# katehai/m-cedm

Hardware: AMD Instinct MI355X
Metric: denoised_states_per_sec_18step_edm_heun (higher is better)
Workload: dtype f32; 1 GPU; SWE-periodic 128x128, EDM U-Net ch=128 ch_mult=[1,1,1,1] attn@16^2 (BASELINE config 3); states_per_gpu=32, global_batch=32, H=128, W=128, sampler=EDM Heun, 18 steps, 35 NFE/state, S_churn=0, w=0, fp64 state / fp32 net, parallelism=batch-sharded x1, no data-path collective, launch=one HIP graph per sampler call

## Files before the change

### include/mcedm_hip.h

```cpp
#ifndef MCEDM_HIP_H_
#define MCEDM_HIP_H_

#include <stddef.h>
#include <stdint.h>

#ifdef __cplusplus
extern "C" {
#endif

#define MCEDM_ABI_VERSION 4
#define MCEDM_REDUCE_SCRATCH_BYTES (4096 * 8 + 64)
#define MCEDM_MAX_LEVELS 8

typedef enum {
  MCEDM_OK = 0,
  MCEDM_ERR_INVALID = -1,
  MCEDM_ERR_UNSUPPORTED = -2,
  MCEDM_ERR_WORKSPACE = -3,
  MCEDM_ERR_HIP = -4
} mcedm_status;

#define MCEDM_DX_NONE 0
#define MCEDM_DX_CAT 1
#define MCEDM_DX_ENC 2
// ... 155 lines not shown
                         const float* init_noise, const double* step_noise, double* out, int return_last, void* workspace,
                         size_t workspace_bytes, int B, int H, int W, void* stream);
int mcedm_vp_heun_sample_rng(const mcedm_plan* plan, const void* packed, const mcedm_vp_sampler_desc* sp, const float* cond,
                             const float* init_noise, const uint64_t* rng_seed, double* out, int return_last, void* workspace,
                             size_t workspace_bytes, int B, int H, int W, void* stream);


typedef struct { float mean, scale, offset, pad; } mcedm_coef;

size_t mcedm_op_conv_packed_floats(int Cout, int Cin, int k);
int mcedm_op_pack_conv(const float* w, const float* b, int Cout, int Cin, int k, int qkv_heads, int dgrad,
                       float* wpk, float* bias_pk, void* stream);
int mcedm_op_gn_coef(const float* xa, const float* xb, int Ca, int Cb, int B, int HW, const float* gamma,
                     const float* beta, const float* film, int film_batch, int film_stride, float eps,
                     mcedm_coef* coef_out, float* stats_out, void* stream);
int mcedm_op_conv(const float* xa, const float* xb, int Ca, int Cb, const mcedm_coef* coef, int coef_batch, int act,
                  int resample, int Hs, int Ws, int H, int W, const float* wpk, const float* bias_pk,
                  const float* res, int res_mode, float* out, int Cout, int B, int k, void* stream);
size_t mcedm_op_conv_wino_packed_floats(int Cout, int Cin);
int mcedm_op_pack_conv_wino(const float* w, int Cout, int Cin, float* wino, void* stream);
int mcedm_op_conv_wino(const float* xa, const float* xb, int Ca, int Cb, const mcedm_coef* coef, int coef_batch, int act,
                       int resample, int H, int W, const float* wino, const float* bias, const float* res, int res_mode,
                       float* out, int Cout, int B, void* stream);
int mcedm_op_embedding(const float* labels, int n, int ch, const float* w0, const float* b0, const float* w1,
                       const float* b1, const float* waff, const float* baff, int rows, float* freqs_scratch,
                       float* emb_out, float* film_out, void* stream);
int mcedm_op_attention(const float* qkv, float* out, int B, int heads, int T, void* stream);
size_t mcedm_op_wgrad_scratch_floats(int Cout, int Cin, int k, int B, int H, int W);
int mcedm_op_conv_wgrad(const float* dy, const float* xa, const float* xb, int Ca, int Cb, const mcedm_coef* coef,
                        int coef_batch, int act, int resample, int Hs, int Ws, int H, int W, int Cout, int B, int k,
                        int qkv_heads, float* scratch, float* dw, float* db, void* stream);
int mcedm_op_gn_bwd(const float* dact, int resample, const float* xa, const float* xb, int Ca, int Cb, int Hs, int Ws,
                    int B, const mcedm_coef* coef, const float* stats, const float* gamma, const float* beta,
                    const float* film, int film_batch, int film_stride, int act, float* dxa, float* dxb, int accumulate,
                    const float* add, int add_mode, float* ab, float* dgamma, float* dbeta, float* dfilm,
                    int dfilm_stride, void* stream);
#define MCEDM_GN_SYNC_WORDS 130
int mcedm_op_gn_bwd_sync(const float* dact, int resample, const float* xa, const float* xb, int Ca, int Cb, int Hs, int Ws,
                         int B, const mcedm_coef* coef, const float* stats, const float* gamma, const float* beta,
                         const float* film, int film_batch, int film_stride, int act, float* dxa, float* dxb, int accumulate,
                         const float* add, int add_mode, float* ab, float* dgamma, float* dbeta, float* dfilm,
                         int dfilm_stride, unsigned int* sync, void* stream);
int mcedm_op_attention_bwd(const float* qkv, const float* a, const float* da, float* dqkv, float* lse_scratch, int B,
                           int heads, int T, void* stream);
int mcedm_op_set_conv_tile(int mt, int ph, int pw);
int mcedm_op_set_conv8(int enable);
int mcedm_op_set_conv_resident(int enable);
int mcedm_op_set_conv_wino(int enable);
int mcedm_op_set_conv_wino1(int enable);
int mcedm_op_set_wgrad_wino(int enable);
int mcedm_op_set_conv1x1_reg(int enable);
int mcedm_op_set_attn_fused(int enable);
int mcedm_op_set_conv_debug(unsigned long long* buf);

typedef struct {
  int32_t in_channels;
  int32_t out_channels;
  int32_t ch;
  int32_t n_levels;
  int32_t ch_mult[MCEDM_MAX_LEVELS];
  int32_t num_res_blocks;
  int32_t resolution;
  int32_t n_attn_resolutions;
  int32_t attn_resolutions[MCEDM_MAX_LEVELS];
  int32_t self_cond;
  float eps;
} mcedm_ddpm_desc;

typedef struct {
  int32_t timesteps;
  double sigma_min, sigma_max, rho;
  double S_churn, S_min, S_max, S_noise;
// ... 65 lines not shown
```

### m-cedm_amd/csrc/conv_wino.hip

```cpp
#include <atomic>
#include <cstdlib>

#include "conv_wino.hpp"
#include "pack.hpp"
#include "prof.hpp"

namespace mcedm {

__global__ void wino_pack_kernel(const float* __restrict__ w, float* __restrict__ dst, int Cout, int Cin, int coutp, int nch,
                                 int tflip) {
  const int idx = blockIdx.x * blockDim.x + threadIdx.x;
  if (idx >= coutp * nch * WKC) return;
  wino_pack_elem(w, dst, idx, Cout, Cin, coutp, tflip);
}

template <class C, bool UP, bool ACT = true>
__global__ __launch_bounds__(C::NT, C::MB == 4 ? 1 : 2) void conv_wino_kernel(const ConvArgs p, int tiles_x, int tiles_img, int nch, int mblocks,
                                                                          int per, int mode) {
  constexpr int WSC = C::SC, VBUF = C::VBUF, RBUF = C::RBUF, MB = C::MB;
  extern __shared__ float lds[];
  const int Cin = p.Ca + p.Cb;
  float* const vbuf = lds;
  float* const rbuf = lds + 2 * VBUF;
  Coef* const cfl = reinterpret_cast<Coef*>(lds + C::LDS_ROWS_OFF);
  float* const xch = lds + C::LDS_ROWS_OFF + 4 * Cin;
  float* const red = xch + C::XCH_FLOATS;
  float* const bias_l = red + 2 * (C::MT / 2) * 3;
  const int tid = threadIdx.x, lane = tid & 63;
  const int wave = __builtin_amdgcn_readfirstlane(tid >> 6);
  const int mb = wave % MB, hf = wave / MB;
  if (p.dbg && tid == 0) { p.dbg[blockIdx.x * 16 + 0] = __builtin_amdgcn_s_memrealtime(); p.dbg[blockIdx.x * 16 + 4] = per; }
  int gt0 = blockIdx.x * per, tstep = 1;
  int n = gt0 / tiles_img, tile0 = gt0 % tiles_img;
  if (mode & 256) {
    const int nwg = gridDim.x, wps = tiles_img / per;
    const int lid = (nwg % 8 == 0) ? (int)(blockIdx.x % 8) * (nwg / 8) + (int)(blockIdx.x / 8) : (int)blockIdx.x;
    n = lid / wps; tile0 = lid % wps; tstep = wps;
  }
  const int m0 = blockIdx.y * C::MT;
  const size_t HW = (size_t)p.H * p.W, HWs = (size_t)p.Hs * p.Ws;
  const int nst = (nch + WSC - 1) / WSC;
// ... 109 lines not shown
        const float* b = rb + sc * WKC * RPLANE + 2 * MB * ti * RPITCH + 2 * j;
        td[sc][ti][0][j] = *reinterpret_cast<const f32x2*>(b + tr_yz);
        td[sc][ti][1][j] = *reinterpret_cast<const f32x2*>(b + tr_yz + RPITCH);
        td[sc][ti][2][j] = *reinterpret_cast<const f32x2*>(b + tr_x);
      }
  };
  auto transform_finish1 = [&](int sc, float* vb) {
#pragma unroll
    for (int ti = 0; ti < C::TI; ++ti) {
      f32x2 t[2][2];
#pragma unroll
      for (int j = 0; j < 2; ++j) {
        t[0][j] = td[sc][ti][0][j] - td[sc][ti][2][j];
        t[1][j] = td[sc][ti][2][j] + tsgn * td[sc][ti][1][j];
      }
#pragma unroll
      for (int x = 0; x < 2; ++x) {
        const f32x2 o03 = t[x][0] - t[x][1];
        const f32x2 c11 = {t[x][0].y, t[x][0].y}, c22 = {t[x][1].x, t[x][1].x};
        const f32x2 o12 = c11 + tpm * c22;
        float* o = vb + sc * 16 * VPOS + tr_dst + MB * ti * WTX * 4 + 4 * x * VPOS;
        o[0 * VPOS] = o03.x;
        o[1 * VPOS] = o12.x;
        o[2 * VPOS] = o12.y;
        o[3 * VPOS] = o03.y;
      }
    }
  };
  auto transform_read = [&](const float* rb) { for (int sc = 0; sc < WSC; ++sc) transform_read1(sc, rb); };
  auto transform_finish = [&](float* vb) { for (int sc = 0; sc < WSC; ++sc) transform_finish1(sc, vb); };

  stage_coef_rows<C::NT>(p, n, cfl, tid);
  if (tid < C::MT) bias_l[tid] = p.bias ? p.bias[m0 + tid] : 0.f;
  raw_load();
  __syncthreads();
  for (int sc = 0; sc < WSC; ++sc) raw_commit1(sc, rbuf);
  commit_done();
  if (G > 1) { raw_load(); for (int sc = 0; sc < WSC; ++sc) raw_commit1(sc, rbuf + RBUF); commit_done(); }
  if (G > 2) raw_load();
  const size_t ustride = (size_t)mblocks * 16 * 64;
  const f32x4* up = reinterpret_cast<const f32x4*>(p.wino) + ((size_t)(m0 / 32 + mb) * 16 + 8 * hf) * 64 + lane;
  f32x4 ua[8];
#pragma unroll
  for (int q = 0; q < 8; ++q) ua[q] = up[q * 64];
  __syncthreads();
  transform_read(rbuf);
  transform_finish(vbuf);
  f32x16 acc[8];
  auto init_acc = [&]() {
    const f32x16 zero16 = {0.f, 0.f, 0.f, 0.f, 0.f, 0.f, 0.f, 0.f, 0.f, 0.f, 0.f, 0.f, 0.f, 0.f, 0.f, 0.f};
    float z = 0.f;
#pragma unroll
    for (int q = 0; q < 8; ++q) {
      asm volatile("" : "+v"(z));
      acc[q] = __builtin_amdgcn_mfma_f32_32x32x2f32(z, z, zero16, 0, 0, 0);
    }
    if (hf == 0) {
#pragma unroll
      for (int r = 0; r < 16; ++r) acc[5][r] = bias_l[32 * mb + 4 * (lane >> 5) + (r & 3) + 8 * (r >> 2)];
    }
  };
  __syncthreads();
  init_acc();

  const int vrd = (8 * hf) * VPOS + (lane >> 5) * VH1 + (lane & 31) * 4;
  if (p.dbg && tid == 0) { p.dbg[blockIdx.x * 16 + 1] = __builtin_amdgcn_s_memrealtime(); p.dbg[blockIdx.x * 16 + 5] = __builtin_amdgcn_s_memtime(); }
#ifdef MCEDM_WINO_TIMELINE
  unsigned long long ph[5] = {0, 0, 0, 0, 0}, tlast = __builtin_amdgcn_s_memtime();
#define WINO_STAMP(i) { const unsigned long long t_ = __builtin_amdgcn_s_memtime(); ph[i] += t_ - tlast; tlast = t_; }
  unsigned long long sl[8] = {0, 0, 0, 0, 0, 0, 0, 0}, slast = 0;
#define WINO_SLOT(i) { const unsigned long long t_ = __builtin_amdgcn_s_memtime(); sl[(i) & 7] += t_ - slast; slast = t_; }
#define WINO_SLOT0 { slast = __builtin_amdgcn_s_memtime(); }
  unsigned long long ep[6] = {0, 0, 0, 0, 0, 0}, elast = 0;
#define WINO_EP(i) { __builtin_amdgcn_sched_barrier(0); const unsigned long long t_ = __builtin_amdgcn_s_memtime(); if (i) ep[(i) - 1] += t_ - elast; elast = t_; __builtin_amdgcn_sched_barrier(0); }
  const bool no_u = mode & 2;
#else
#define WINO_STAMP(i)
#define WINO_SLOT(i)
#define WINO_SLOT0
#define WINO_EP(i)
  constexpr bool no_u = false;
#endif
  auto side_slice = [&](int slot, int g, int cur) {
    if (WSC == 2) {
      if (slot == 0) transform_read1(0, rbuf + (cur ^ 1) * RBUF);
      if (slot == 1) raw_commit1(0, rbuf + cur * RBUF);
      if (slot == 2) { transform_finish1(0, vbuf + (cur ^ 1) * VBUF); raw_load1(0); }
      if (slot == 3) transform_read1(WSC - 1, rbuf + (cur ^ 1) * RBUF);
      if (slot == 4) { raw_commit1(WSC - 1, rbuf + cur * RBUF); commit_done(); }
      if (slot == 5) { transform_finish1(WSC - 1, vbuf + (cur ^ 1) * VBUF); raw_load1(WSC - 1); raw_load_done(); }
    } else {
      if (slot == 0) transform_read(rbuf + (cur ^ 1) * RBUF);
      if (slot == 1) { raw_commit1(0, rbuf + cur * RBUF); commit_done(); }
      if (slot == 2) { raw_load1(0); raw_load_done(); }
      if (slot == 3) transform_finish1(0, vbuf + (cur ^ 1) * VBUF);
    }
  };
  (void)mode;
  int st = 0, tile = tile0;
  for (int g = 0; g < G; ++g) {
    const int cur = g & 1;
    WINO_STAMP(0)
    WINO_SLOT0
#pragma unroll
    for (int sc = 0; sc < WSC; ++sc) {
      const int c = st * WSC + sc;
      const f32x4* un = up + (size_t)(c + 1 < nch ? c + 1 : 0) * ustride;
      const float* vb = vbuf + cur * VBUF + sc * 16 * VPOS + vrd;
      f32x4 b4[2][2];
      b4[0][0] = *reinterpret_cast<const f32x4*>(vb);
      b4[0][1] = *reinterpret_cast<const f32x4*>(vb + VPOS);
      __builtin_amdgcn_sched_group_barrier(0x100, 2, 0);
#pragma unroll
      for (int qp = 0; qp < 4; ++qp) {
        const int cb = qp & 1;
        if (qp < 3) {
          b4[cb ^ 1][0] = *reinterpret_cast<const f32x4*>(vb + (2 * qp + 2) * VPOS);
          b4[cb ^ 1][1] = *reinterpret_cast<const f32x4*>(vb + (2 * qp + 3) * VPOS);
        }
#pragma unroll
        for (int s = 0; s < 4; ++s) {
          acc[2 * qp] = __builtin_amdgcn_mfma_f32_32x32x2f32(ua[2 * qp][s], b4[cb][0][s], acc[2 * qp], 0, 0, 0);
          acc[2 * qp + 1] = __builtin_amdgcn_mfma_f32_32x32x2f32(ua[2 * qp + 1][s], b4[cb][1][s], acc[2 * qp + 1], 0, 0, 0);
        }
        if (!no_u) {
          ua[2 * qp] = un[(2 * qp) * 64];
          ua[2 * qp + 1] = un[(2 * qp + 1) * 64];
        }
        side_slice(sc * 4 + qp, g, cur);
        if (qp < 3) __builtin_amdgcn_sched_group_barrier(0x100, 2, 0);
#pragma unroll
        for (int i = 0; i < 8; ++i) {
          __builtin_amdgcn_sched_group_barrier(0x008, 1, 0);
          __builtin_amdgcn_sched_group_barrier(0x486, WINO_IL_K, 0);
        }
        __builtin_amdgcn_sched_group_barrier(0x020, 4, 0);
        __builtin_amdgcn_sched_barrier(0);
        if (sc * 4 + qp == (WSC == 2 ? 5 : 2)) raw_load_next();
        __builtin_amdgcn_sched_barrier(0);
        WINO_SLOT(sc * 4 + qp + (WSC == 1 ? 0 : 0))
      }
    }
    WINO_STAMP(1)
    __syncthreads();
    WINO_STAMP(2)
    if (++st < nst) continue;
    st = 0;

    WINO_EP(0)
    const int y0 = (tile / tiles_x) * WPH, x0 = (tile % tiles_x) * WPW;
    const int pt = lane & 31;
    const int oy = y0 + 2 * (pt >> 3) + hf, ox = x0 + 2 * (pt & 7);
    const int cbase = m0 + 32 * mb + 4 * (lane >> 5);
    const size_t splane = (size_t)p.Cout * HW;
    const __amdgpu_buffer_rsrc_t rs_out = make_rsrc(p.out + (size_t)n * splane, 4u * (unsigned)splane);
    const size_t rplane = p.res_mode == RS_UP ? splane >> 2 : p.res_mode == RS_DOWN ? splane << 2 : splane;
    const __amdgpu_buffer_rsrc_t rs_res = make_rsrc(p.res ? p.res + (size_t)n * rplane : nullptr, p.res ? 4u * (unsigned)rplane : 0u);
    const unsigned HWu = (unsigned)HW;
    const unsigned voff = 4u * ((unsigned)cbase * HWu + (unsigned)oy * p.W + ox);
    const unsigned rvoff = 4u * ((unsigned)cbase * (HWu >> 2) + (unsigned)(oy >> 1) * (p.W >> 1) + (ox >> 1));
    float2 rv[16];
    f32x16 keep[2], send[2];
#pragma unroll
    for (int j = 0; j < 2; ++j) {
      const f32x16 t0 = j == 0 ? acc[0] + acc[1] + acc[2] : acc[1] - acc[2] - acc[3];
      const f32x16 t1 = j == 0 ? acc[4] + acc[5] + acc[6] : acc[5] - acc[6] - acc[7];
      if (hf == 0) { keep[j] = t0 + t1; send[j] = t1; }
      else         { keep[j] = -t0 - t1; send[j] = t0; }
      __builtin_amdgcn_sched_barrier(0);
    }
    __builtin_amdgcn_sched_barrier(0);
    if (p.res && p.res_mode == RS_DOWN) {
      const unsigned dvoff = 4u * ((unsigned)cbase * (HWu << 2) + (unsigned)(2 * oy) * (unsigned)(2 * p.W) + (unsigned)(2 * ox));
#pragma unroll
      for (int r0 = 0; r0 < 16; r0 += 4) {
        f32x4 ta[4], tb[4];
#pragma unroll
        for (int k = 0; k < 4; ++k) {
          const unsigned so = 4u * (unsigned)(((r0 + k) & 3) + 8 * ((r0 + k) >> 2)) * (HWu << 2);
          ta[k] = __builtin_bit_cast(f32x4, __builtin_amdgcn_raw_buffer_load_b128(rs_res, dvoff, so, 0));
          tb[k] = __builtin_bit_cast(f32x4, __builtin_amdgcn_raw_buffer_load_b128(rs_res, dvoff + 8u * (unsigned)p.W, so, 0));
        }
#pragma unroll
        for (int k = 0; k < 4; ++k)
          rv[r0 + k] = make_float2(0.25f * ((ta[k][0] + ta[k][1]) + (tb[k][0] + tb[k][1])), 0.25f * ((ta[k][2] + ta[k][3]) + (tb[k][2] + tb[k][3])));
      }
    } else {
#pragma unroll
      for (int r = 0; r < 16; ++r) {
// ... 63 lines not shown
        }
      }
      __syncthreads();
      conv_stats_store<C, 2>(p, red, n, m0, tile, tiles_img, tid);
    }
    WINO_EP(4)
    __builtin_amdgcn_sched_barrier(0);
    init_acc();
    tile += tstep;
    WINO_EP(5)
    WINO_STAMP(3)
  }
  if (p.dbg && tid == 0) {
    asm volatile("s_waitcnt vmcnt(0)" ::: "memory");
    p.dbg[blockIdx.x * 16 + 2] = __builtin_amdgcn_s_memrealtime(); p.dbg[blockIdx.x * 16 + 6] = __builtin_amdgcn_s_memtime();
    p.dbg[blockIdx.x * 16 + 3] = __builtin_amdgcn_s_memrealtime();
  }
#ifdef MCEDM_WINO_TIMELINE
  if (p.dbg && tid == 0) for (int i = 0; i < 5; ++i) p.dbg[blockIdx.x * 16 + 8 + i] = ph[i];
  if (p.dbg && tid == 0 && (mode & 16)) for (int i = 0; i < 8; ++i) p.dbg[blockIdx.x * 16 + 8 + i] = sl[i];
  if (p.dbg && tid == 0 && (mode & 32)) for (int i = 0; i < 6; ++i) p.dbg[blockIdx.x * 16 + 8 + i] = ep[i];
  if (p.dbg && tid == 64 * MB && !(mode & 48)) { p.dbg[blockIdx.x * 16 + 13] = ph[1]; p.dbg[blockIdx.x * 16 + 14] = ph[2]; p.dbg[blockIdx.x * 16 + 15] = ph[3]; p.dbg[blockIdx.x * 16 + 7] = ph[0]; }
#endif
}

static int g_wino = -1;
void set_conv_wino(int enable) { g_wino = enable; }
static int wino_env() {
  static int env = -1;
  if (env < 0) { const char* e = getenv("MCEDM_WINOGRAD"); env = e ? atoi(e) : 1; }
  return variant_choice(KV_CONV_WINO, g_wino, env);
}
static int wino_mode_env() {
  static int env = -1;
  if (env < 0) {
    const char* e = getenv("MCEDM_WINO_MODE");
    const char* m = getenv("MCEDM_WINO_MAP");
    env = ((e ? atoi(e) : 0) & ~256) | ((m ? atoi(m) : 1) ? 256 : 0);
  }
  return env;
}

static int wino_min_hw_env() {
  static int env = -1;
  if (env < 0) { const char* e = getenv("MCEDM_WINO_MIN_HW"); env = e ? atoi(e) : 1024; }
  return env;
// ... 29 lines not shown
  return best;
}

template <class C>
static int launch_wino_cfg(const ConvArgs& a, hipStream_t stream) {
  const int tiles_x = a.W / WPW, tiles_img = tiles_x * (a.H / WPH);
  const long long total = (long long)a.B * tiles_img;
  MCEDM_REQUIRE(total > 0 && total <= 0x7fffffffLL, "conv_wino: grid out of range");
  const int Cin = a.Ca + a.Cb, nch = Cin / WKC;
  const int lds_bytes = (C::LDS_ROWS_OFF + 4 * Cin + C::XCH_FLOATS + C::RED_FLOATS) * 4;
  MCEDM_REQUIRE(lds_bytes <= 160 * 1024 / (C::MB == 4 ? 1 : 2), "conv_wino: %d input channels exceed the LDS row table", Cin);
  static std::atomic<bool> attr_set[64];
  static std::atomic<int> ncu[64];
  int dev = 0;
  MCEDM_HIP_TRY(hipGetDevice(&dev));
  MCEDM_REQUIRE(dev >= 0 && dev < 64, "device index %d out of range", dev);
  if (!attr_set[dev].load(std::memory_order_acquire)) {
    int n_cu = 0;
    MCEDM_HIP_TRY(hipDeviceGetAttribute(&n_cu, hipDeviceAttributeMultiprocessorCount, dev));
    ncu[dev].store(n_cu > 0 ? n_cu : 256, std::memory_order_release);
    MCEDM_HIP_TRY(hipFuncSetAttribute((const void*)conv_wino_kernel<C, false>, hipFuncAttributeMaxDynamicSharedMemorySize, 160 * 1024));
    MCEDM_HIP_TRY(hipFuncSetAttribute((const void*)conv_wino_kernel<C, true>, hipFuncAttributeMaxDynamicSharedMemorySize, 160 * 1024));
    MCEDM_HIP_TRY(hipFuncSetAttribute((const void*)conv_wino_kernel<C, false, false>, hipFuncAttributeMaxDynamicSharedMemorySize, 160 * 1024));
    attr_set[dev].store(true, std::memory_order_release);
  }
  static int per_env = -1;
  if (per_env < 0) { const char* e = getenv("MCEDM_WINO_PER"); per_env = e ? atoi(e) : 0; }
  int per = wino_tiles_per_wg(total, tiles_img, ncu[dev].load(std::memory_order_acquire) * (C::MB == 4 ? 1 : 2));
  if (per_env > 0 && tiles_img % per_env == 0) per = per_env;
  char name[64] = "";
  const bool noact = a.resample != RS_UP && !a.act;
  if (prof_enabled()) snprintf(name, sizeof(name), "conv_wino_kernel<WinoCfg<%d>, %s, %s>", C::MB, a.resample == RS_UP ? "true" : "false",
                               noact ? "false" : "true");
  const double px = (double)a.B * a.H * a.W;
  ProfScope ps(name, 2.0 * px * a.Cout * (double)Cin * 9,
               4.0 * ((double)a.B * Cin * a.Hs * a.Ws + px * a.Cout * (a.res ? 2 : 1) + (double)a.Cout * Cin * 9), stream);
  if (a.resample == RS_UP)
    hipLaunchKernelGGL((conv_wino_kernel<C, true>), dim3((unsigned)(total / per), a.Cout / C::MT), dim3(C::NT), lds_bytes, stream, a, tiles_x,
                       tiles_img, nch, cout_padded(a.Cout) / 32, per, wino_mode_env());
  else if (noact)
    hipLaunchKernelGGL((conv_wino_kernel<C, false, false>), dim3((unsigned)(total / per), a.Cout / C::MT), dim3(C::NT), lds_bytes, stream, a, tiles_x,
                       tiles_img, nch, cout_padded(a.Cout) / 32, per, wino_mode_env());
  else
    hipLaunchKernelGGL((conv_wino_kernel<C, false>), dim3((unsigned)(total / per), a.Cout / C::MT), dim3(C::NT), lds_bytes, stream, a, tiles_x,
                       tiles_img, nch, cout_padded(a.Cout) / 32, per, wino_mode_env());
  MCEDM_LAUNCH_CHECK("conv_wino_kernel");
  if (a.gsum_tiles) *a.gsum_tiles = SumTiles{tiles_img, tiles_x, WPH, WPW, a.gsum_rc == 2 ? 2 : 4};
  return MCEDM_OK;
}

int launch_conv_wino(const ConvArgs& a_in, hipStream_t stream) {
  ConvArgs a = a_in;
  a.dbg = conv_debug_buffer();
  MCEDM_REQUIRE(conv_wino_applicable(a, 9), "conv_wino: shape not served by the Winograd kernel");
  MCEDM_REQUIRE(a.out && a.B > 0 && (a.resample == RS_UP ? (a.Hs * 2 == a.H && a.Ws * 2 == a.W) : (a.Hs == a.H && a.Ws == a.W)),
                "conv_wino: bad arguments");
  MCEDM_REQUIRE((unsigned long long)a.H * a.W * 4ull * a.Cout * (a.res && a.res_mode == RS_DOWN ? 4 : 1) < (1ull << 32),
                "conv_wino: one sample of the output / residual exceeds the 4 GiB buffer range");
  { const int rc = conv_resolve_identity(a); if (rc != MCEDM_OK) return rc; }
  if (a.Cout % 128 == 0) {
// ... 13 lines not shown
```

### m-cedm_amd/csrc/conv_wino.hpp

```cpp
#pragma once
#include "conv_tile.hpp"

namespace mcedm {

constexpr int WPH = 8, WPW = 16;
constexpr int WTX = WPW / 2, WTY = WPH / 2;
constexpr int WKC = 8;
static_assert(WTX * WTY == 32, "one MFMA N block of patches per workgroup");
template <int MB_>
struct WinoCfg {
  static constexpr int MB = MB_, NT = 128 * MB_, NW = 2 * MB_, MT = 32 * MB_;
  static constexpr int SC = MB_ == 4 ? 2 : 1;
  static constexpr int CPW = WKC / NW;
  static constexpr int TI = 4 / MB_;
  static constexpr int VBUF = SC * 16 * 288, RBUF = SC * WKC * 196;
  static constexpr int LDS_ROWS_OFF = 2 * VBUF + 2 * RBUF;
  static constexpr int XCH_FLOATS = NW * 16 * 64;
  static constexpr int RED_FLOATS = 2 * (MT / 2) * 3 + MT;
  static_assert(MB_ == 4 || MB_ == 2, "128 or 64 output channels per workgroup");
  static_assert(LDS_ROWS_OFF % 4 == 0, "LDS layout");
};
constexpr int RROWS = WPH + 2, RPITCH = WPW + 2;
constexpr int RPLANE = 196;
constexpr int RSUB = (RROWS * RPITCH + 63) / 64;
constexpr int WINO_IL_K = 5;
constexpr int VH1 = 144, VPOS = 288;
static_assert(RPLANE % 32 == 4 && VH1 % 32 == 16 && VH1 >= 128 && VPOS >= VH1 + 128 && RPLANE >= RROWS * RPITCH && RPLANE % 2 == 0 && VPOS % 4 == 0 && VH1 % 4 == 0, "LDS layout");



int try_launch_conv_wino1(const ConvArgs& a, hipStream_t stream);
void set_conv_wino1(int enable);
int wino_tiles_per_wg(long long total, int tiles_img, int slots);

}
```

### m-cedm_amd/csrc/ops_api.hip

```cpp
#include "common.hpp"
#include "conv_wino.hpp"
#include "bwd.hpp"

using namespace mcedm;

static_assert(sizeof(mcedm_coef) == sizeof(Coef), "mcedm_coef must mirror Coef");

extern "C" size_t mcedm_op_conv_packed_floats(int Cout, int Cin, int k) {
  if (Cout <= 0 || Cin <= 0 || (k != 1 && k != 3)) return 0;
  return conv_packed_floats(Cout, Cin, k * k);
}

extern "C" int mcedm_op_pack_conv(const float* w, const float* b, int Cout, int Cin, int k, int qkv_heads, int dgrad,
                                  float* wpk, float* bias_pk, void* stream) {
  MCEDM_REQUIRE(w && wpk, "op_pack_conv: null pointer");
  MCEDM_REQUIRE(Cout > 0 && Cin > 0 && (k == 1 || k == 3), "op_pack_conv: bad shape");
  MCEDM_REQUIRE(qkv_heads == 0 || (Cout % (3 * qkv_heads) == 0 && !dgrad), "op_pack_conv: bad qkv_heads");
  int rc = dgrad ? launch_pack_conv(w, wpk, Cin, Cout, k * k, 0, 1, (hipStream_t)stream)
                 : launch_pack_conv(w, wpk, Cout, Cin, k * k, qkv_heads, 0, (hipStream_t)stream);
  if (rc) return rc;
  if (b && bias_pk) rc = launch_pack_bias(b, bias_pk, Cout, qkv_heads, (hipStream_t)stream);
  return rc;
}

// ... 10 lines not shown
}

extern "C" int mcedm_op_conv(const float* xa, const float* xb, int Ca, int Cb, const mcedm_coef* coef, int coef_batch,
                             int act, int resample, int Hs, int Ws, int H, int W, const float* wpk,
                             const float* bias_pk, const float* res, int res_mode, float* out, int Cout, int B, int k,
                             void* stream) {
  MCEDM_REQUIRE(k == 1 || k == 3, "op_conv: k must be 1 or 3");
  MCEDM_REQUIRE(resample >= 0 && resample <= 3 && res_mode >= 0 && res_mode <= 2, "op_conv: bad resample mode");
  ConvArgs a{};
  a.xa = xa; a.xb = xb; a.Ca = Ca; a.Cb = Cb;
  a.coef = reinterpret_cast<const Coef*>(coef); a.coef_batch = coef_batch; a.act = act;
  a.resample = resample; a.Hs = Hs; a.Ws = Ws; a.H = H; a.W = W;
  a.wpk = wpk; a.bias = bias_pk; a.res = res; a.res_mode = res_mode;
  a.out = out; a.Cout = Cout; a.B = B;
  return launch_conv(a, k * k, (hipStream_t)stream);
}

extern "C" size_t mcedm_op_conv_wino_packed_floats(int Cout, int Cin) { return conv_wino_packed_floats(Cout, Cin); }

extern "C" int mcedm_op_pack_conv_wino(const float* w, int Cout, int Cin, float* wino, void* stream) {
  return launch_pack_conv_wino(w, wino, Cout, Cin, 0, (hipStream_t)stream);
}

extern "C" int mcedm_op_conv_wino(const float* xa, const float* xb, int Ca, int Cb, const mcedm_coef* coef, int coef_batch,
                                  int act, int resample, int H, int W, const float* wino, const float* bias, const float* res,
                                  int res_mode, float* out, int Cout, int B, void* stream) {
  MCEDM_REQUIRE((resample == RS_NONE || resample == RS_UP) && (res_mode == RS_NONE || res_mode == RS_UP || res_mode == RS_DOWN),
                "op_conv_wino: resample must be 0 (none) or 1 (nearest-2x up), res_mode 0, 1 or 2 (2x2-mean down)");
  ConvArgs a{};
  a.xa = xa; a.xb = xb; a.Ca = Ca; a.Cb = Cb;
  a.coef = reinterpret_cast<const Coef*>(coef); a.coef_batch = coef_batch; a.act = act;
  a.resample = resample; a.H = H; a.W = W;
  a.Hs = resample == RS_UP ? H / 2 : H; a.Ws = resample == RS_UP ? W / 2 : W;
  a.wino = wino; a.bias = bias; a.res = res; a.res_mode = res_mode;
  a.out = out; a.Cout = Cout; a.B = B;
  MCEDM_REQUIRE(conv_wino_applicable(a, 9), "op_conv_wino: needs Cout %% 64 == 0, H %% 8 == 0, W %% 16 == 0, Cin %% 8 == 0 and 16-byte aligned inputs / weight table");
  return launch_conv_wino(a, (hipStream_t)stream);
}

__global__ void op_freqs_kernel(float* f, int half) {
  const int k = blockIdx.x * blockDim.x + threadIdx.x;
  if (k < half) f[k] = powf(1.0f / 10000.0f, (float)k / (float)half);
}

extern "C" int mcedm_op_embedding(const float* labels, int n, int ch, const float* w0, const float* b0, const float* w1,
                                  const float* b1, const float* waff, const float* baff, int rows, float* freqs_scratch,
                                  float* emb_out, float* film_out, void* stream) {
  MCEDM_REQUIRE(labels && w0 && b0 && w1 && b1 && waff && baff && freqs_scratch && film_out, "op_embedding: null pointer");
  MCEDM_REQUIRE(n > 0 && ch > 0 && ch % 2 == 0 && rows > 0, "op_embedding: bad shape n=%d ch=%d rows=%d", n, ch, rows);
  hipLaunchKernelGGL(op_freqs_kernel, dim3(ceil_div(ch / 2, 64)), dim3(64), 0, (hipStream_t)stream, freqs_scratch, ch / 2);
  MCEDM_LAUNCH_CHECK("op_freqs_kernel");
  EmbArgs e{labels, n, ch, freqs_scratch, w0, b0, w1, b1, waff, baff, rows, emb_out, film_out};
  return launch_embedding(e, (hipStream_t)stream);
}

extern "C" int mcedm_op_attention(const float* qkv, float* out, int B, int heads, int T, void* stream) {
  MCEDM_REQUIRE(qkv && out, "op_attention: null pointer");
  return launch_attention(qkv, out, B, heads, T, (hipStream_t)stream);
}

// ... 54 lines not shown
                        accumulate, add, add_mode, ab, dgamma, dbeta, dfilm, dfilm_stride, sync, stream);
}

extern "C" int mcedm_op_attention_bwd(const float* qkv, const float* a, const float* da, float* dqkv, float* lse_scratch,
                                      int B, int heads, int T, void* stream) {
  return launch_attention_bwd(qkv, a, da, dqkv, lse_scratch, B, heads, T, (hipStream_t)stream);
}

extern "C" int mcedm_op_set_conv8(int enable) {
  set_conv8(enable);
  return MCEDM_OK;
}

extern "C" int mcedm_op_set_conv_wino(int enable) {
  set_conv_wino(enable);
  return MCEDM_OK;
}

extern "C" int mcedm_op_set_conv_wino1(int enable) {
  set_conv_wino1(enable);
  return MCEDM_OK;
}

extern "C" int mcedm_op_set_conv1x1_reg(int enable) {
  set_conv1x1_reg(enable);
  return MCEDM_OK;
}

extern "C" int mcedm_op_set_wgrad_wino(int enable) {
  set_wgrad_wino(enable);
  return MCEDM_OK;
}

extern "C" int mcedm_op_set_conv_resident(int enable) {
  set_conv_resident(enable);
  return MCEDM_OK;
}

extern "C" int mcedm_op_set_attn_fused(int enable) {
  set_attn_fused(enable);
  return MCEDM_OK;
}

extern "C" int mcedm_op_set_conv_debug(unsigned long long* buf) {
  set_conv_debug(buf);
  return MCEDM_OK;
// ... 2 lines not shown
```

### m-cedm_amd/lib.py

```python
from __future__ import annotations

import ctypes as C
import os
from typing import Dict, List, Optional, Sequence

import torch

_HERE = os.path.dirname(os.path.abspath(__file__))
LIB_PATH = os.environ.get("MCEDM_LIB") or os.path.join(_HERE, "libmcedm_hip.so")
MAX_LEVELS = 8

EXPORTS = [
    "mcedm_version", "mcedm_last_error", "mcedm_unet_plan_create", "mcedm_unet_plan_destroy",
    "mcedm_unet_param_count", "mcedm_unet_param_info", "mcedm_unet_packed_bytes", "mcedm_unet_pack_weights",
    "mcedm_unet_workspace_bytes", "mcedm_unet_forward", "mcedm_edm_denoise", "mcedm_sampler_workspace_bytes",
    "mcedm_heun_sample", "mcedm_edm_t_steps", "mcedm_edm_loss", "mcedm_edm_noise_inputs",
    "mcedm_edm_denoise_backward", "mcedm_edm_denoise_backward_bucketed", "mcedm_unet_grad_buckets", "mcedm_sqnorm",
    "mcedm_adam_ema_step",
    "mcedm_swe_fv_step", "mcedm_swe_fv_residual", "mcedm_darcy_residual", "mcedm_swe_fv_guidance", "mcedm_darcy_guidance",
    "mcedm_heun_sample_guided",
    "mcedm_ddpm_plan_create", "mcedm_ddpm_plan_destroy", "mcedm_ddpm_param_count", "mcedm_ddpm_param_info",
    "mcedm_ddpm_packed_bytes", "mcedm_ddpm_pack_weights", "mcedm_ddpm_workspace_bytes", "mcedm_ddpm_forward",
    "mcedm_ddpm_denoise", "mcedm_repaint_schedule", "mcedm_repaint_workspace_bytes", "mcedm_repaint_sample",
    "mcedm_repaint_sample_rng", "mcedm_normal_fill", "mcedm_ddpm_forward_sc", "mcedm_ddim_workspace_bytes",
# ... 882 lines not shown
        return lib
    vp, i32, sz = C.c_void_p, C.c_int, C.c_size_t
    lib.mcedm_op_conv_packed_floats.argtypes = [i32, i32, i32]
    lib.mcedm_op_conv_packed_floats.restype = sz
    lib.mcedm_op_pack_conv.argtypes = [vp, vp, i32, i32, i32, i32, i32, vp, vp, vp]
    lib.mcedm_op_gn_coef.argtypes = [vp, vp, i32, i32, i32, i32, vp, vp, vp, i32, i32, C.c_float, vp, vp, vp]
    lib.mcedm_op_conv.argtypes = [vp, vp, i32, i32, vp, i32, i32, i32, i32, i32, i32, i32, vp, vp, vp, i32, vp, i32,
                                  i32, i32, vp]
    lib.mcedm_op_attention.argtypes = [vp, vp, i32, i32, i32, vp]
    lib.mcedm_op_embedding.argtypes = [vp, i32, i32, vp, vp, vp, vp, vp, vp, i32, vp, vp, vp, vp]
    lib.mcedm_op_wgrad_scratch_floats.argtypes = [i32, i32, i32, i32, i32, i32]
    lib.mcedm_op_wgrad_scratch_floats.restype = sz
    lib.mcedm_op_conv_wgrad.argtypes = [vp, vp, vp, i32, i32, vp, i32, i32, i32, i32, i32, i32, i32, i32, i32, i32, i32,
                                        vp, vp, vp, vp]
    lib.mcedm_op_gn_bwd.argtypes = [vp, i32, vp, vp, i32, i32, i32, i32, i32, vp, vp, vp, vp, vp, i32, i32, i32, vp, vp,
                                    i32, vp, i32, vp, vp, vp, vp, i32, vp]
    lib.mcedm_op_gn_bwd_sync.argtypes = [vp, i32, vp, vp, i32, i32, i32, i32, i32, vp, vp, vp, vp, vp, i32, i32, i32, vp, vp,
                                         i32, vp, i32, vp, vp, vp, vp, i32, vp, vp]
    lib.mcedm_op_attention_bwd.argtypes = [vp, vp, vp, vp, vp, i32, i32, i32, vp]
    lib.mcedm_op_conv_wino_packed_floats.argtypes = [i32, i32]
    lib.mcedm_op_conv_wino_packed_floats.restype = sz
    lib.mcedm_op_pack_conv_wino.argtypes = [vp, i32, i32, vp, vp]
    lib.mcedm_op_conv_wino.argtypes = [vp, vp, i32, i32, vp, i32, i32, i32, i32, i32, vp, vp, vp, i32, vp, i32, i32, vp]
    for n in ("mcedm_op_pack_conv", "mcedm_op_gn_coef", "mcedm_op_conv", "mcedm_op_attention", "mcedm_op_embedding", "mcedm_op_conv_wgrad",
              "mcedm_op_gn_bwd", "mcedm_op_gn_bwd_sync", "mcedm_op_attention_bwd", "mcedm_op_pack_conv_wino", "mcedm_op_conv_wino"):
        getattr(lib, n).restype = C.c_int
    _OPS_BOUND = True
    return lib


OP_EXPORTS = ["mcedm_op_conv_packed_floats", "mcedm_op_pack_conv", "mcedm_op_gn_coef", "mcedm_op_conv",
              "mcedm_op_attention", "mcedm_op_set_conv_tile", "mcedm_prof_enable", "mcedm_prof_report",
              "mcedm_op_wgrad_scratch_floats", "mcedm_op_conv_wgrad", "mcedm_op_gn_bwd", "mcedm_op_attention_bwd",
              "mcedm_op_set_conv_debug", "mcedm_op_set_conv8", "mcedm_op_set_conv_resident", "mcedm_op_set_attn_fused", "mcedm_op_embedding",
              "mcedm_op_conv_wino_packed_floats", "mcedm_op_pack_conv_wino", "mcedm_op_conv_wino", "mcedm_op_set_conv_wino", "mcedm_op_set_conv_wino1",
              "mcedm_op_set_wgrad_wino", "mcedm_op_set_conv1x1_reg", "mcedm_op_gn_bwd_sync"]


def prof_enable(on: bool) -> None:
    lib = load()
    lib.mcedm_prof_enable.argtypes = [C.c_int]
    check(lib.mcedm_prof_enable(int(on)), "prof_enable")


def prof_report() -> list:
    import json
    lib = load()
    lib.mcedm_prof_report.argtypes = [C.c_char_p, C.c_size_t]
    buf = C.create_string_buffer(1 << 16)
    check(lib.mcedm_prof_report(buf, len(buf)), "prof_report")
    return json.loads(buf.value.decode())


def set_conv_tile(mt: int = 0, ph: int = 0, pw: int = 0) -> None:
    lib = _bind_ops()
    lib.mcedm_op_set_conv_tile.argtypes = [C.c_int, C.c_int, C.c_int]
    check(lib.mcedm_op_set_conv_tile(mt, ph, pw), "set_conv_tile")
def set_conv8(enable: int = -1) -> None:
    lib = _bind_ops()
    lib.mcedm_op_set_conv8.argtypes = [C.c_int]
    check(lib.mcedm_op_set_conv8(int(enable)), "set_conv8")


def set_conv_wino(enable: int = -1) -> None:
    lib = _bind_ops()
    lib.mcedm_op_set_conv_wino.argtypes = [C.c_int]
    check(lib.mcedm_op_set_conv_wino(int(enable)), "set_conv_wino")


def set_conv_wino1(enable: int = -1) -> None:
    lib = _bind_ops()
    lib.mcedm_op_set_conv_wino1.argtypes = [C.c_int]
    check(lib.mcedm_op_set_conv_wino1(int(enable)), "set_conv_wino1")


def set_conv1x1_reg(enable: int = -1) -> None:
    lib = _bind_ops()
    lib.mcedm_op_set_conv1x1_reg.argtypes = [C.c_int]
    check(lib.mcedm_op_set_conv1x1_reg(int(enable)), "set_conv1x1_reg")


def set_wgrad_wino(enable: int = -1) -> None:
    lib = _bind_ops()
    lib.mcedm_op_set_wgrad_wino.argtypes = [C.c_int]
    check(lib.mcedm_op_set_wgrad_wino(int(enable)), "set_wgrad_wino")


def set_conv_resident(enable: int = -1) -> None:
    lib = _bind_ops()
    lib.mcedm_op_set_conv_resident.argtypes = [C.c_int]
    check(lib.mcedm_op_set_conv_resident(int(enable)), "set_conv_resident")


def set_attn_fused(enable: int = -1) -> None:
    lib = _bind_ops()
    lib.mcedm_op_set_attn_fused.argtypes = [C.c_int]
# ... 40 lines not shown
                            _ptr(bias_pk), _ptr(res), res_mode, _ptr(out), Cout, B, k, _stream()), "op_conv")
    return out


def op_pack_conv_wino(w: torch.Tensor) -> torch.Tensor:
    lib = _bind_ops()
    Cout, Cin = w.shape[:2]
    wino = torch.empty(lib.mcedm_op_conv_wino_packed_floats(Cout, Cin), dtype=torch.float32, device=w.device)
    check(lib.mcedm_op_pack_conv_wino(_ptr(w), Cout, Cin, _ptr(wino), _stream()), "op_pack_conv_wino")
    return wino


def op_conv_wino(xa, xb, wino, bias, Cout, coef=None, coef_batch=1, act=0, resample=RS_NONE, res=None, res_mode=RS_NONE,
                 out=None):
    lib = _bind_ops()
    B, Ca, Hs, Ws = xa.shape
    Cb = xb.shape[1] if xb is not None else 0
    H, W = (Hs * 2, Ws * 2) if resample == RS_UP else (Hs, Ws)
    if out is None:
        out = torch.empty((B, Cout, H, W), dtype=torch.float32, device=xa.device)
    check(lib.mcedm_op_conv_wino(_ptr(xa), _ptr(xb), Ca, Cb, _ptr(coef), coef_batch, act, resample, H, W, _ptr(wino),
                                 _ptr(bias), _ptr(res), res_mode, _ptr(out), Cout, B, _stream()), "op_conv_wino")
    return out


def op_embedding(labels, w0, b0, w1, b1, waff, baff):
    lib = _bind_ops()
    n, ch, rows = labels.numel(), w0.shape[0], waff.shape[0]
    freqs = torch.empty(ch // 2, dtype=torch.float32, device=labels.device)
    emb = torch.empty((n, ch), dtype=torch.float32, device=labels.device)
    film = torch.empty((n, rows), dtype=torch.float32, device=labels.device)
    check(lib.mcedm_op_embedding(_ptr(labels), n, ch, _ptr(w0), _ptr(b0), _ptr(w1), _ptr(b1), _ptr(waff), _ptr(baff), rows,
                                 _ptr(freqs), _ptr(emb), _ptr(film), _stream()), "op_embedding")
    return emb, film


def op_attention(qkv: torch.Tensor, heads: int) -> torch.Tensor:
    lib = _bind_ops()
    B, C3, H, W = qkv.shape
    out = torch.empty((B, C3 // 3, H, W), dtype=torch.float32, device=qkv.device)
    check(lib.mcedm_op_attention(_ptr(qkv), _ptr(out), B, heads, H * W, _stream()), "op_attention")
    return out


def op_conv_wgrad(dy, xa, xb, k, coef=None, coef_batch=1, act=0, resample=RS_NONE, qkv_heads=0):
    lib = _bind_ops()
# ... 44 lines not shown
```

Baseline: 78.40 states/s.

## Skip structurally zero Winograd products in upsampled conv kernel

Adds a sparse path to the Winograd conv kernel for nearest-2x upsampled inputs. Nearest upsampling makes some transformed input rows zero, so the kernel skips the matching MFMA products, weight loads and LDS stores, and one half-wave's work entirely. The old dense path stays reachable through a new env/setter toggle. A stats-emitting conv entry point is also exposed. The change adds schedule complexity and uneven work across waves.

Result: faster. 80.58 states/s (median of 6 runs) (+2.8%).

```diff
diff --git a/include/mcedm_hip.h b/include/mcedm_hip.h
--- a/include/mcedm_hip.h
+++ b/include/mcedm_hip.h
@@ -201,6 +201,9 @@
 int mcedm_op_conv_wino(const float* xa, const float* xb, int Ca, int Cb, const mcedm_coef* coef, int coef_batch, int act,
                        int resample, int H, int W, const float* wino, const float* bias, const float* res, int res_mode,
                        float* out, int Cout, int B, void* stream);
+int mcedm_op_conv_wino_stats(const float* xa, const float* xb, int Ca, int Cb, const mcedm_coef* coef, int coef_batch, int act,
+                             int resample, int H, int W, const float* wino, const float* bias, const float* res, int res_mode,
+                             float* out, int Cout, int B, float* gsum, int gsum_rc, void* stream);
 int mcedm_op_embedding(const float* labels, int n, int ch, const float* w0, const float* b0, const float* w1,
                        const float* b1, const float* waff, const float* baff, int rows, float* freqs_scratch,
                        float* emb_out, float* film_out, void* stream);
@@ -227,6 +230,7 @@
 int mcedm_op_set_conv_resident(int enable);
 int mcedm_op_set_conv_wino(int enable);
 int mcedm_op_set_conv_wino1(int enable);
+int mcedm_op_set_conv_wino_up_dense(int enable);
 int mcedm_op_set_wgrad_wino(int enable);
 int mcedm_op_set_conv1x1_reg(int enable);
 int mcedm_op_set_attn_fused(int enable);
diff --git a/m-cedm_amd/csrc/conv_wino.hip b/m-cedm_amd/csrc/conv_wino.hip
--- a/m-cedm_amd/csrc/conv_wino.hip
+++ b/m-cedm_amd/csrc/conv_wino.hip
@@ -17,6 +17,7 @@
 template <class C, bool UP, bool ACT = true>
 __global__ __launch_bounds__(C::NT, C::MB == 4 ? 1 : 2) void conv_wino_kernel(const ConvArgs p, int tiles_x, int tiles_img, int nch, int mblocks,
                                                                           int per, int mode) {
+  constexpr bool SP = UP && !C::UP_DENSE;
   constexpr int WSC = C::SC, VBUF = C::VBUF, RBUF = C::RBUF, MB = C::MB;
   extern __shared__ float lds[];
   const int Cin = p.Ca + p.Cb;
@@ -172,7 +173,7 @@
         float* o = vb + sc * 16 * VPOS + tr_dst + MB * ti * WTX * 4 + 4 * x * VPOS;
         o[0 * VPOS] = o03.x;
         o[1 * VPOS] = o12.x;
-        o[2 * VPOS] = o12.y;
+        if (!SP) o[2 * VPOS] = o12.y;
         o[3 * VPOS] = o03.y;
       }
     }
@@ -192,7 +193,8 @@
   const f32x4* up = reinterpret_cast<const f32x4*>(p.wino) + ((size_t)(m0 / 32 + mb) * 16 + 8 * hf) * 64 + lane;
   f32x4 ua[8];
 #pragma unroll
-  for (int q = 0; q < 8; ++q) ua[q] = up[q * 64];
+  for (int q = 0; q < 8; ++q)
+    if (!SP || ((q & 3) != 2 && !(hf == 1 && q < 4))) ua[q] = up[q * 64];
   __syncthreads();
   transform_read(rbuf);
   transform_finish(vbuf);
@@ -202,6 +204,7 @@
     float z = 0.f;
 #pragma unroll
     for (int q = 0; q < 8; ++q) {
+      if (SP && (q & 3) == 2) continue;
       asm volatile("" : "+v"(z));
       acc[q] = __builtin_amdgcn_mfma_f32_32x32x2f32(z, z, zero16, 0, 0, 0);
     }
@@ -232,7 +235,20 @@
   constexpr bool no_u = false;
 #endif
   auto side_slice = [&](int slot, int g, int cur) {
-    if (WSC == 2) {
+    if (SP) {
+      if (WSC == 2) {
+        if (slot == 0) transform_read1(0, rbuf + (cur ^ 1) * RBUF);
+        if (slot == 2) raw_commit1(0, rbuf + cur * RBUF);
+        if (slot == 3) { transform_finish1(0, vbuf + (cur ^ 1) * VBUF); raw_load1(0); }
+        if (slot == 4) transform_read1(WSC - 1, rbuf + (cur ^ 1) * RBUF);
+        if (slot == 6) { raw_commit1(WSC - 1, rbuf + cur * RBUF); commit_done(); }
+        if (slot == 7) { transform_finish1(WSC - 1, vbuf + (cur ^ 1) * VBUF); raw_load1(WSC - 1); raw_load_done(); }
+      } else {
+        if (slot == 0) transform_read(rbuf + (cur ^ 1) * RBUF);
+        if (slot == 2) { raw_commit1(0, rbuf + cur * RBUF); commit_done(); }
+        if (slot == 3) { transform_finish1(0, vbuf + (cur ^ 1) * VBUF); raw_load1(0); raw_load_done(); }
+      }
+    } else if (WSC == 2) {
       if (slot == 0) transform_read1(0, rbuf + (cur ^ 1) * RBUF);
       if (slot == 1) raw_commit1(0, rbuf + cur * RBUF);
       if (slot == 2) { transform_finish1(0, vbuf + (cur ^ 1) * VBUF); raw_load1(0); }
@@ -247,6 +263,7 @@
     }
   };
   (void)mode;
+  const bool xdead = SP && hf == 1;
   int st = 0, tile = tile0;
   for (int g = 0; g < G; ++g) {
     const int cur = g & 1;
@@ -258,35 +275,66 @@
       const f32x4* un = up + (size_t)(c + 1 < nch ? c + 1 : 0) * ustride;
       const float* vb = vbuf + cur * VBUF + sc * 16 * VPOS + vrd;
       f32x4 b4[2][2];
-      b4[0][0] = *reinterpret_cast<const f32x4*>(vb);
-      b4[0][1] = *reinterpret_cast<const f32x4*>(vb + VPOS);
-      __builtin_amdgcn_sched_group_barrier(0x100, 2, 0);
+      if (!xdead) {
+        b4[0][0] = *reinterpret_cast<const f32x4*>(vb);
+        b4[0][1] = *reinterpret_cast<const f32x4*>(vb + VPOS);
+      }
+      if (!SP) __builtin_amdgcn_sched_group_barrier(0x100, 2, 0);
 #pragma unroll
       for (int qp = 0; qp < 4; ++qp) {
         const int cb = qp & 1;
-        if (qp < 3) {
-          b4[cb ^ 1][0] = *reinterpret_cast<const f32x4*>(vb + (2 * qp + 2) * VPOS);
-          b4[cb ^ 1][1] = *reinterpret_cast<const f32x4*>(vb + (2 * qp + 3) * VPOS);
-        }
-#pragma unroll
-        for (int s = 0; s < 4; ++s) {
-          acc[2 * qp] = __builtin_amdgcn_mfma_f32_32x32x2f32(ua[2 * qp][s], b4[cb][0][s], acc[2 * qp], 0, 0, 0);
-          acc[2 * qp + 1] = __builtin_amdgcn_mfma_f32_32x32x2f32(ua[2 * qp + 1][s], b4[cb][1][s], acc[2 * qp + 1], 0, 0, 0);
-        }
-        if (!no_u) {
-          ua[2 * qp] = un[(2 * qp) * 64];
-          ua[2 * qp + 1] = un[(2 * qp + 1) * 64];
-        }
-        side_slice(sc * 4 + qp, g, cur);
-        if (qp < 3) __builtin_amdgcn_sched_group_barrier(0x100, 2, 0);
-#pragma unroll
-        for (int i = 0; i < 8; ++i) {
-          __builtin_amdgcn_sched_group_barrier(0x008, 1, 0);
-          __builtin_amdgcn_sched_group_barrier(0x486, WINO_IL_K, 0);
+        const bool l0 = !SP || !(qp & 1), n0 = !SP || (qp & 1);
+        if (!SP || qp >= 2) {
+          if (qp < 3) {
+            if (n0) b4[cb ^ 1][0] = *reinterpret_cast<const f32x4*>(vb + (2 * qp + 2) * VPOS);
+            b4[cb ^ 1][1] = *reinterpret_cast<const f32x4*>(vb + (2 * qp + 3) * VPOS);
+          }
+#pragma unroll
+          for (int s = 0; s < 4; ++s) {
+            if (l0) acc[2 * qp] = __builtin_amdgcn_mfma_f32_32x32x2f32(ua[2 * qp][s], b4[cb][0][s], acc[2 * qp], 0, 0, 0);
+            acc[2 * qp + 1] = __builtin_amdgcn_mfma_f32_32x32x2f32(ua[2 * qp + 1][s], b4[cb][1][s], acc[2 * qp + 1], 0, 0, 0);
+          }
+          if (!no_u) {
+            if (l0) ua[2 * qp] = un[(2 * qp) * 64];
+            ua[2 * qp + 1] = un[(2 * qp + 1) * 64];
+          }
+          side_slice(sc * 4 + qp, g, cur);
+          if (qp < 3) { if (n0) __builtin_amdgcn_sched_group_barrier(0x100, 2, 0); else __builtin_amdgcn_sched_group_barrier(0x100, 1, 0); }
+          if (l0) {
+#pragma unroll
+            for (int i = 0; i < 8; ++i) {
+              __builtin_amdgcn_sched_group_barrier(0x008, 1, 0);
+              __builtin_amdgcn_sched_group_barrier(0x486, WINO_IL_K, 0);
+            }
+          } else {
+#pragma unroll
+            for (int i = 0; i < 4; ++i) {
+              __builtin_amdgcn_sched_group_barrier(0x008, 1, 0);
+              __builtin_amdgcn_sched_group_barrier(0x486, WINO_IL_K4, 0);
+            }
+          }
+        } else {
+          if (qp == 1) {
+            b4[0][0] = *reinterpret_cast<const f32x4*>(vb + 4 * VPOS);
+            b4[0][1] = *reinterpret_cast<const f32x4*>(vb + 5 * VPOS);
+          }
+          side_slice(sc * 4 + qp, g, cur);
+          if (!xdead) {
+            if (qp == 0) b4[1][1] = *reinterpret_cast<const f32x4*>(vb + 3 * VPOS);
+#pragma unroll
+            for (int s = 0; s < 4; ++s) {
+              if (l0) acc[2 * qp] = __builtin_amdgcn_mfma_f32_32x32x2f32(ua[2 * qp][s], b4[cb][0][s], acc[2 * qp], 0, 0, 0);
+              acc[2 * qp + 1] = __builtin_amdgcn_mfma_f32_32x32x2f32(ua[2 * qp + 1][s], b4[cb][1][s], acc[2 * qp + 1], 0, 0, 0);
+            }
+            if (!no_u) {
+              if (l0) ua[2 * qp] = un[(2 * qp) * 64];
+              ua[2 * qp + 1] = un[(2 * qp + 1) * 64];
+            }
+          }
         }
         __builtin_amdgcn_sched_group_barrier(0x020, 4, 0);
         __builtin_amdgcn_sched_barrier(0);
-        if (sc * 4 + qp == (WSC == 2 ? 5 : 2)) raw_load_next();
+        if (sc * 4 + qp == (SP ? WSC * 4 - 1 : WSC == 2 ? 5 : 2)) raw_load_next();
         __builtin_amdgcn_sched_barrier(0);
         WINO_SLOT(sc * 4 + qp + (WSC == 1 ? 0 : 0))
       }
@@ -313,8 +361,15 @@
     f32x16 keep[2], send[2];
 #pragma unroll
     for (int j = 0; j < 2; ++j) {
-      const f32x16 t0 = j == 0 ? acc[0] + acc[1] + acc[2] : acc[1] - acc[2] - acc[3];
-      const f32x16 t1 = j == 0 ? acc[4] + acc[5] + acc[6] : acc[5] - acc[6] - acc[7];
+      const f32x16 z16 = {0.f, 0.f, 0.f, 0.f, 0.f, 0.f, 0.f, 0.f, 0.f, 0.f, 0.f, 0.f, 0.f, 0.f, 0.f, 0.f};
+      f32x16 t0, t1;
+      if constexpr (SP) {
+        t0 = j == 0 ? acc[0] + acc[1] + z16 : acc[1] - z16 - acc[3];
+        t1 = j == 0 ? acc[4] + acc[5] + z16 : acc[5] - z16 - acc[7];
+      } else {
+        t0 = j == 0 ? acc[0] + acc[1] + acc[2] : acc[1] - acc[2] - acc[3];
+        t1 = j == 0 ? acc[4] + acc[5] + acc[6] : acc[5] - acc[6] - acc[7];
+      }
       if (hf == 0) { keep[j] = t0 + t1; send[j] = t1; }
       else         { keep[j] = -t0 - t1; send[j] = t0; }
       __builtin_amdgcn_sched_barrier(0);
@@ -424,6 +479,14 @@
   if (p.dbg && tid == 0 && (mode & 32)) for (int i = 0; i < 6; ++i) p.dbg[blockIdx.x * 16 + 8 + i] = ep[i];
   if (p.dbg && tid == 64 * MB && !(mode & 48)) { p.dbg[blockIdx.x * 16 + 13] = ph[1]; p.dbg[blockIdx.x * 16 + 14] = ph[2]; p.dbg[blockIdx.x * 16 + 15] = ph[3]; p.dbg[blockIdx.x * 16 + 7] = ph[0]; }
 #endif
+}
+
+static int g_wino_up_dense = -1;
+void set_conv_wino_up_dense(int enable) { g_wino_up_dense = enable; }
+static bool wino_up_dense() {
+  static int env = -1;
+  if (env < 0) { const char* e = getenv("MCEDM_WINO_UP_DENSE"); env = e ? (atoi(e) != 0) : 0; }
+  return g_wino_up_dense >= 0 ? g_wino_up_dense != 0 : env != 0;
 }
 
 static int g_wino = -1;
@@ -499,6 +562,7 @@
     MCEDM_HIP_TRY(hipFuncSetAttribute((const void*)conv_wino_kernel<C, false>, hipFuncAttributeMaxDynamicSharedMemorySize, 160 * 1024));
     MCEDM_HIP_TRY(hipFuncSetAttribute((const void*)conv_wino_kernel<C, true>, hipFuncAttributeMaxDynamicSharedMemorySize, 160 * 1024));
     MCEDM_HIP_TRY(hipFuncSetAttribute((const void*)conv_wino_kernel<C, false, false>, hipFuncAttributeMaxDynamicSharedMemorySize, 160 * 1024));
+    MCEDM_HIP_TRY(hipFuncSetAttribute((const void*)conv_wino_kernel<WinoUpDense<C::MB>, true>, hipFuncAttributeMaxDynamicSharedMemorySize, 160 * 1024));
     attr_set[dev].store(true, std::memory_order_release);
   }
   static int per_env = -1;
@@ -507,12 +571,18 @@
   if (per_env > 0 && tiles_img % per_env == 0) per = per_env;
   char name[64] = "";
   const bool noact = a.resample != RS_UP && !a.act;
-  if (prof_enabled()) snprintf(name, sizeof(name), "conv_wino_kernel<WinoCfg<%d>, %s, %s>", C::MB, a.resample == RS_UP ? "true" : "false",
-                               noact ? "false" : "true");
+  const bool up_dense = a.resample == RS_UP && wino_up_dense();
+  if (prof_enabled()) {
+    if (up_dense) snprintf(name, sizeof(name), "conv_wino_kernel<WinoUpDense<%d>, true, true>", C::MB);
+    else snprintf(name, sizeof(name), "conv_wino_kernel<WinoCfg<%d>, %s, %s>", C::MB, a.resample == RS_UP ? "true" : "false", noact ? "false" : "true");
+  }
   const double px = (double)a.B * a.H * a.W;
   ProfScope ps(name, 2.0 * px * a.Cout * (double)Cin * 9,
                4.0 * ((double)a.B * Cin * a.Hs * a.Ws + px * a.Cout * (a.res ? 2 : 1) + (double)a.Cout * Cin * 9), stream);
-  if (a.resample == RS_UP)
+  if (up_dense)
+    hipLaunchKernelGGL((conv_wino_kernel<WinoUpDense<C::MB>, true>), dim3((unsigned)(total / per), a.Cout / C::MT), dim3(C::NT), lds_bytes, stream, a, tiles_x,
+                       tiles_img, nch, cout_padded(a.Cout) / 32, per, wino_mode_env());
+  else if (a.resample == RS_UP)
     hipLaunchKernelGGL((conv_wino_kernel<C, true>), dim3((unsigned)(total / per), a.Cout / C::MT), dim3(C::NT), lds_bytes, stream, a, tiles_x,
                        tiles_img, nch, cout_padded(a.Cout) / 32, per, wino_mode_env());
   else if (noact)
diff --git a/m-cedm_amd/csrc/conv_wino.hpp b/m-cedm_amd/csrc/conv_wino.hpp
--- a/m-cedm_amd/csrc/conv_wino.hpp
+++ b/m-cedm_amd/csrc/conv_wino.hpp
@@ -17,13 +17,19 @@
   static constexpr int LDS_ROWS_OFF = 2 * VBUF + 2 * RBUF;
   static constexpr int XCH_FLOATS = NW * 16 * 64;
   static constexpr int RED_FLOATS = 2 * (MT / 2) * 3 + MT;
+  static constexpr bool UP_DENSE = false;
   static_assert(MB_ == 4 || MB_ == 2, "128 or 64 output channels per workgroup");
   static_assert(LDS_ROWS_OFF % 4 == 0, "LDS layout");
+};
+template <int MB_>
+struct WinoUpDense : WinoCfg<MB_> {
+  static constexpr bool UP_DENSE = true;
 };
 constexpr int RROWS = WPH + 2, RPITCH = WPW + 2;
 constexpr int RPLANE = 196;
 constexpr int RSUB = (RROWS * RPITCH + 63) / 64;
 constexpr int WINO_IL_K = 5;
+constexpr int WINO_IL_K4 = 8;
 constexpr int VH1 = 144, VPOS = 288;
 static_assert(RPLANE % 32 == 4 && VH1 % 32 == 16 && VH1 >= 128 && VPOS >= VH1 + 128 && RPLANE >= RROWS * RPITCH && RPLANE % 2 == 0 && VPOS % 4 == 0 && VH1 % 4 == 0, "LDS layout");
 
@@ -31,6 +37,7 @@
 
 int try_launch_conv_wino1(const ConvArgs& a, hipStream_t stream);
 void set_conv_wino1(int enable);
+void set_conv_wino_up_dense(int enable);
 int wino_tiles_per_wg(long long total, int tiles_img, int slots);
 
 }
diff --git a/m-cedm_amd/csrc/ops_api.hip b/m-cedm_amd/csrc/ops_api.hip
--- a/m-cedm_amd/csrc/ops_api.hip
+++ b/m-cedm_amd/csrc/ops_api.hip
@@ -56,9 +56,9 @@
   return launch_pack_conv_wino(w, wino, Cout, Cin, 0, (hipStream_t)stream);
 }
 
-extern "C" int mcedm_op_conv_wino(const float* xa, const float* xb, int Ca, int Cb, const mcedm_coef* coef, int coef_batch,
-                                  int act, int resample, int H, int W, const float* wino, const float* bias, const float* res,
-                                  int res_mode, float* out, int Cout, int B, void* stream) {
+static int op_conv_wino_impl(const float* xa, const float* xb, int Ca, int Cb, const mcedm_coef* coef, int coef_batch, int act, int resample,
+                             int H, int W, const float* wino, const float* bias, const float* res, int res_mode, float* out, int Cout, int B,
+                             float* gsum, int gsum_rc, void* stream) {
   MCEDM_REQUIRE((resample == RS_NONE || resample == RS_UP) && (res_mode == RS_NONE || res_mode == RS_UP || res_mode == RS_DOWN),
                 "op_conv_wino: resample must be 0 (none) or 1 (nearest-2x up), res_mode 0, 1 or 2 (2x2-mean down)");
   ConvArgs a{};
@@ -68,8 +68,22 @@
   a.Hs = resample == RS_UP ? H / 2 : H; a.Ws = resample == RS_UP ? W / 2 : W;
   a.wino = wino; a.bias = bias; a.res = res; a.res_mode = res_mode;
   a.out = out; a.Cout = Cout; a.B = B;
+  a.gsum = gsum; a.gsum_rc = gsum_rc;
   MCEDM_REQUIRE(conv_wino_applicable(a, 9), "op_conv_wino: needs Cout %% 64 == 0, H %% 8 == 0, W %% 16 == 0, Cin %% 8 == 0 and 16-byte aligned inputs / weight table");
   return launch_conv_wino(a, (hipStream_t)stream);
+}
+
+extern "C" int mcedm_op_conv_wino(const float* xa, const float* xb, int Ca, int Cb, const mcedm_coef* coef, int coef_batch,
+                                  int act, int resample, int H, int W, const float* wino, const float* bias, const float* res,
+                                  int res_mode, float* out, int Cout, int B, void* stream) {
+  return op_conv_wino_impl(xa, xb, Ca, Cb, coef, coef_batch, act, resample, H, W, wino, bias, res, res_mode, out, Cout, B, nullptr, 0, stream);
+}
+
+extern "C" int mcedm_op_conv_wino_stats(const float* xa, const float* xb, int Ca, int Cb, const mcedm_coef* coef, int coef_batch,
+                                        int act, int resample, int H, int W, const float* wino, const float* bias, const float* res,
+                                        int res_mode, float* out, int Cout, int B, float* gsum, int gsum_rc, void* stream) {
+  MCEDM_REQUIRE(gsum && (gsum_rc == 4 || gsum_rc == 2), "op_conv_wino_stats: needs a statistics table and 4 or 2 channels per record");
+  return op_conv_wino_impl(xa, xb, Ca, Cb, coef, coef_batch, act, resample, H, W, wino, bias, res, res_mode, out, Cout, B, gsum, gsum_rc, stream);
 }
 
 __global__ void op_freqs_kernel(float* f, int half) {
@@ -170,6 +184,11 @@
   return MCEDM_OK;
 }
 
+extern "C" int mcedm_op_set_conv_wino_up_dense(int enable) {
+  set_conv_wino_up_dense(enable);
+  return MCEDM_OK;
+}
+
 extern "C" int mcedm_op_set_conv1x1_reg(int enable) {
   set_conv1x1_reg(enable);
   return MCEDM_OK;
diff --git a/m-cedm_amd/lib.py b/m-cedm_amd/lib.py
--- a/m-cedm_amd/lib.py
+++ b/m-cedm_amd/lib.py
@@ -928,6 +928,8 @@
     lib.mcedm_op_conv_wino_packed_floats.restype = sz
     lib.mcedm_op_pack_conv_wino.argtypes = [vp, i32, i32, vp, vp]
     lib.mcedm_op_conv_wino.argtypes = [vp, vp, i32, i32, vp, i32, i32, i32, i32, i32, vp, vp, vp, i32, vp, i32, i32, vp]
+    lib.mcedm_op_conv_wino_stats.argtypes = [vp, vp, i32, i32, vp, i32, i32, i32, i32, i32, vp, vp, vp, i32, vp, i32, i32, vp, i32, vp]
+    lib.mcedm_op_conv_wino_stats.restype = C.c_int
     for n in ("mcedm_op_pack_conv", "mcedm_op_gn_coef", "mcedm_op_conv", "mcedm_op_attention", "mcedm_op_embedding", "mcedm_op_conv_wgrad",
               "mcedm_op_gn_bwd", "mcedm_op_gn_bwd_sync", "mcedm_op_attention_bwd", "mcedm_op_pack_conv_wino", "mcedm_op_conv_wino"):
         getattr(lib, n).restype = C.c_int
@@ -940,6 +942,7 @@
               "mcedm_op_wgrad_scratch_floats", "mcedm_op_conv_wgrad", "mcedm_op_gn_bwd", "mcedm_op_attention_bwd",
               "mcedm_op_set_conv_debug", "mcedm_op_set_conv8", "mcedm_op_set_conv_resident", "mcedm_op_set_attn_fused", "mcedm_op_embedding",
               "mcedm_op_conv_wino_packed_floats", "mcedm_op_pack_conv_wino", "mcedm_op_conv_wino", "mcedm_op_set_conv_wino", "mcedm_op_set_conv_wino1",
+              "mcedm_op_set_conv_wino_up_dense", "mcedm_op_conv_wino_stats",
               "mcedm_op_set_wgrad_wino", "mcedm_op_set_conv1x1_reg", "mcedm_op_gn_bwd_sync"]
 
 
@@ -978,6 +981,12 @@
     lib = _bind_ops()
     lib.mcedm_op_set_conv_wino1.argtypes = [C.c_int]
     check(lib.mcedm_op_set_conv_wino1(int(enable)), "set_conv_wino1")
+
+
+def set_conv_wino_up_dense(enable: int = -1) -> None:
+    lib = _bind_ops()
+    lib.mcedm_op_set_conv_wino_up_dense.argtypes = [C.c_int]
+    check(lib.mcedm_op_set_conv_wino_up_dense(int(enable)), "set_conv_wino_up_dense")
 
 
 def set_conv1x1_reg(enable: int = -1) -> None:
@@ -1064,6 +1073,18 @@
     check(lib.mcedm_op_conv_wino(_ptr(xa), _ptr(xb), Ca, Cb, _ptr(coef), coef_batch, act, resample, H, W, _ptr(wino),
                                  _ptr(bias), _ptr(res), res_mode, _ptr(out), Cout, B, _stream()), "op_conv_wino")
     return out
+
+
+def op_conv_wino_stats(xa, xb, wino, bias, Cout, coef=None, coef_batch=1, act=0, resample=RS_NONE, res=None, res_mode=RS_NONE, rc=4):
+    lib = _bind_ops()
+    B, Ca, Hs, Ws = xa.shape
+    Cb = xb.shape[1] if xb is not None else 0
+    H, W = (Hs * 2, Ws * 2) if resample == RS_UP else (Hs, Ws)
+    out = torch.empty((B, Cout, H, W), dtype=torch.float32, device=xa.device)
+    gsum = torch.zeros((B, (H // 8) * (W // 16), Cout // rc, 2), dtype=torch.float32, device=xa.device)
+    check(lib.mcedm_op_conv_wino_stats(_ptr(xa), _ptr(xb), Ca, Cb, _ptr(coef), coef_batch, act, resample, H, W, _ptr(wino),
+                                       _ptr(bias), _ptr(res), res_mode, _ptr(out), Cout, B, _ptr(gsum), rc, _stream()), "op_conv_wino_stats")
+    return out, gsum
 
 
 def op_embedding(labels, w0, b0, w1, b1, waff, baff):
```
